# dalek-cryptography/zkp

Measured on AMD Instinct MI355X. Metric: proofs/sec + batch-verifies/sec, CMZ13 10-attr credential, 1/2/4/8 MI355X, higher is better.
Workload: dtype u32x9 (29-bit limbs, u64 accumulate)

## Files before the change

include/zkp_mi355x.h:

```cpp
#ifndef ZKP_MI355X_H
#define ZKP_MI355X_H

#include <stddef.h>
#include <stdint.h>

#ifdef __cplusplus
extern "C" {
#endif

#define ZKP_OK 0
#define ZKP_ERR_HIP (-1)
#define ZKP_ERR_ARG (-2)
#define ZKP_ERR_NO_DEVICE (-3)
#define ZKP_ERR_OOM (-4)

#define ZKP_VARTIME 0
#define ZKP_CT 1

typedef struct zkp_ctx zkp_ctx;

int zkp_ctx_create(zkp_ctx** out, int device_id);
void zkp_ctx_destroy(zkp_ctx* ctx);
int zkp_ctx_set_stream(zkp_ctx* ctx, void* hip_stream);
int zkp_ctx_synchronize(zkp_ctx* ctx);
const char* zkp_last_error(void);
const char* zkp_version(void);

enum { ZKP_OPT_BATCH_ENCODE_MIN = 1, ZKP_OPT_COMB_TEETH = 2, ZKP_OPT_CT_SINGLE_USE_TABLES = 3, ZKP_OPT_TRANSCRIPT_LANES = 4, ZKP_OPT_DEV_OVERLAP = 5, ZKP_OPT_GROUPED_COMB = 6, ZKP_OPT_TABLES_LANE = 7,
       ZKP_OPT_FUSE_TABLES_TRANSCRIPT = 8, ZKP_OPT_CT_LOOKUP = 9, ZKP_OPT_CT_MASKED_SCANS = 9 , ZKP_OPT_EACH_STRAUS = 10, ZKP_OPT_LADDER_INTERLEAVE = 11, ZKP_OPT_WS_LIMIT_BYTES = 12, ZKP_OPT_JOB_DEFER_D2H = 13, ZKP_OPT_SYNC_SCHEDULE = 14, ZKP_OPT_TRANSCRIPT_STEPS = 15, ZKP_OPT_COMB_SPLIT = 16, ZKP_OPT_JOINT_LADDER = 17 };
int zkp_ctx_set_option(zkp_ctx* ctx, int option, uint64_t value);

typedef struct zkp_graph zkp_graph;
int zkp_ctx_capture_begin(zkp_ctx* ctx);
int zkp_ctx_capture_end(zkp_ctx* ctx, zkp_graph** out);
int zkp_ctx_capture_abort(zkp_ctx* ctx);
int zkp_graph_launch(zkp_graph* graph, zkp_ctx* ctx);
void zkp_graph_destroy(zkp_graph* graph);

int zkp_ctx_prepare_fixed_points(zkp_ctx* ctx, uint32_t n, const uint8_t* encodings);

int zkp_msm_many(zkp_ctx* ctx, uint32_t n_msm, const uint32_t* off, const uint8_t* scalars ,
                 const uint32_t* pidx , const uint8_t* points , uint32_t n_points,
                 int flags, uint8_t* out , uint8_t* status );
int zkp_msm_many_dev(zkp_ctx* ctx, uint32_t n_msm, const uint32_t* d_off, const uint8_t* d_scalars,
                     const uint32_t* d_pidx, const uint8_t* d_points, uint32_t n_points, uint32_t n_terms,
                     int flags, uint8_t* d_out, uint8_t* d_status);

int zkp_msm_optional(zkp_ctx* ctx, uint64_t n, const uint8_t* scalars ,
                     const uint8_t* points , uint8_t out_point[32], int* status);
int zkp_msm_optional_dev(zkp_ctx* ctx, uint64_t n, const uint8_t* d_scalars, const uint8_t* d_points,
                         uint8_t* d_out_point , uint32_t* d_status );

// ... 288 lines not shown
```

rust/zkp-mi355x-sys/src/lib.rs:

```rust
#![allow(non_camel_case_types)]
use std::os::raw::{c_char, c_int, c_void};

#[repr(C)]
pub struct zkp_ctx {
    _private: [u8; 0],
}
#[repr(C)]
pub struct zkp_graph {
    _private: [u8; 0],
}
#[repr(C)]
pub struct zkp_statement {
    _private: [u8; 0],
}
#[repr(C)]
pub struct zkp_pipe {
    _private: [u8; 0],
}
#[repr(C)]
pub struct zkp_job {
    _private: [u8; 0],
}

pub const ZKP_OK: c_int = 0;
// ... 8 lines not shown
pub const ZKP_DLOG_FOUND: u8 = 0;
pub const ZKP_DLOG_INVALID: u8 = 1;
pub const ZKP_DLOG_NOT_FOUND: u8 = 2;
pub const ZKP_DLOG_SLOTS: u32 = 8;
pub const ZKP_DLOG_SIGNED: c_int = 1;
pub const ZKP_OPT_BATCH_ENCODE_MIN: c_int = 1;
pub const ZKP_OPT_COMB_TEETH: c_int = 2;
pub const ZKP_OPT_CT_SINGLE_USE_TABLES: c_int = 3;
pub const ZKP_OPT_TRANSCRIPT_LANES: c_int = 4;
pub const ZKP_OPT_DEV_OVERLAP: c_int = 5;
pub const ZKP_OPT_GROUPED_COMB: c_int = 6;
pub const ZKP_OPT_TABLES_LANE: c_int = 7;
pub const ZKP_OPT_FUSE_TABLES_TRANSCRIPT: c_int = 8;
pub const ZKP_OPT_CT_LOOKUP: c_int = 9;
pub const ZKP_OPT_CT_MASKED_SCANS: c_int = 9;
pub const ZKP_OPT_EACH_STRAUS: c_int = 10;
pub const ZKP_OPT_LADDER_INTERLEAVE: c_int = 11;
pub const ZKP_OPT_WS_LIMIT_BYTES: c_int = 12;
pub const ZKP_OPT_JOB_DEFER_D2H: c_int = 13;
pub const ZKP_OPT_SYNC_SCHEDULE: c_int = 14;
pub const ZKP_OPT_TRANSCRIPT_STEPS: c_int = 15;
pub const ZKP_OPT_COMB_SPLIT: c_int = 16;
pub const ZKP_OPT_JOINT_LADDER: c_int = 17;
pub const ZKP_JOB_SHARED_TRANSCRIPT: u32 = 1;

pub const ZKP_TB_OK: c_int = 0;
pub const ZKP_TB_VERIFICATION_FAILURE: c_int = 1;
pub const ZKP_TB_BATCH_SIZE_MISMATCH: c_int = 2;
pub const ZKP_TB_PIPE_FULL: c_int = 3;
pub const ZKP_TB_BAD_STATEMENT: c_int = -10;
pub const ZKP_TB_INVALID_POINT: c_int = -11;
pub const ZKP_TB_NO_ENTROPY: c_int = -12;
pub const ZKP_TB_BAD_ENCODING: c_int = -13;
pub const ZKP_TRANSCRIPT_BYTES: usize = 208;

#[repr(C)]
pub struct zkp_batch_statement {
    pub n_secrets: u32,
    pub n_static: u32,
    pub n_instance: u32,
    pub n_constraints: u32,
    pub cons_lhs: *const u32,
    pub cons_off: *const u32,
    pub cons_sc: *const u32,
    pub cons_pt: *const u32,
}
// ... 373 lines not shown
```

zkp_amd/csrc/ge25519.h:

```cpp
#pragma once
#include "fe25519.h"
#include "fe_constants.h"

namespace zkp {

struct ge_p3 { fe X, Y, Z, T; };
struct ge_cached { fe YpX, YmX, Z2, T2d; };
struct ge_niels { fe ypx, ymx, xy2d; };

ZKP_HD void ge_identity(ge_p3& r) {
  fe_0(r.X);
  fe_1(r.Y);
  fe_1(r.Z);
  fe_0(r.T);
}
ZKP_HD void ge_cached_identity(ge_cached& r) {
  fe_1(r.YpX);
  fe_1(r.YmX);
  fe_0(r.Z2);
  r.Z2.v[0] = 2;
  FE_TRACK(fe_set_ub_exact(r.Z2));
  fe_0(r.T2d);
}
ZKP_HD void ge_niels_identity(ge_niels& r) {
// ... 206 lines not shown
  fe_cmov(q.T2d, n, flag);
}
ZKP_HD void ge_niels_cneg(ge_niels& q, uint32_t flag) {
  fe_cswap(q.ypx, q.ymx, flag);
  fe n;
  fe_neg(n, q.xy2d);
  fe_cmov(q.xy2d, n, flag);
}
ZKP_HD void ge_cached_cmov(ge_cached& r, const ge_cached& q, uint32_t flag) {
  fe_cmov(r.YpX, q.YpX, flag);
  fe_cmov(r.YmX, q.YmX, flag);
  fe_cmov(r.Z2, q.Z2, flag);
  fe_cmov(r.T2d, q.T2d, flag);
}

ZKP_HD uint32_t fe_words_eq(const uint32_t w[8], const fe_words& c) {
  uint32_t x = 0;
#pragma unroll
  for (int i = 0; i < 8; ++i) x |= w[i] ^ c.w[i];
  return (uint32_t)(x == 0);
}

ZKP_HD uint32_t fe_invsqrt(fe& r, const fe& v) {
  fe t, v3, c;
  fe_sq(t, v);
  fe_mul(v3, t, v);
  fe_sq(t, v3);
  fe_mul(t, t, v);
  fe_pow22523(t, t);
  fe_mul(r, t, v3);
  fe_sq(t, r);
  fe_mul(t, t, v);
  uint32_t cw[8];
  fe_towords(cw, t);
  const uint32_t correct = fe_words_eq(cw, FE_W_ONE);
  const uint32_t flipped = fe_words_eq(cw, FE_W_MINUS_ONE);
  const uint32_t flipped_i = fe_words_eq(cw, FE_W_MINUS_SQRT_M1);
  fe_from_const(c, FE_SQRT_M1);
  fe_mul(t, r, c);
  fe_cmov(r, t, flipped | flipped_i);
  fe_abs(r, r);
  return correct | flipped;
}

ZKP_HD uint32_t fe_words_eq(const uint32_t a[8], const uint32_t b[8]) {
  uint32_t x = 0;
#pragma unroll
  for (int i = 0; i < 8; ++i) x |= a[i] ^ b[i];
  return (uint32_t)(x == 0);
}

ZKP_HD uint32_t fe_sqrt_ratio_m1(fe& r, const fe& u, const fe& v) {
  fe t, v3, c;
// ... 226 lines not shown
```

zkp_amd/csrc/zkp_kernels.hip:

```cpp
#include <hip/hip_runtime.h>
#include <sys/syscall.h>
#include <unistd.h>
#include <cctype>
#include <cstdio>
#include <cstring>
#include <algorithm>
#include <atomic>
#include <functional>
#include <map>
#include <memory>
#include <mutex>
#include <set>
#include <string>
#include <unordered_map>
#include <vector>
#include "../../include/zkp_mi355x.h"
#include "dev_layout.h"

using namespace zkp;

__device__ __forceinline__ uint32_t sel8(const uint32_t w[8], int j) {
  uint32_t r = w[0];
#pragma unroll
  for (int i = 1; i < 8; ++i) r = (j == i) ? w[i] : r;
// ... 589 lines not shown
           uint8_t* __restrict__ status) {
  const uint32_t b = blockIdx.x * blockDim.x + threadIdx.x;
  if (b >= K) return;
  const uint32_t sg = pip_csr_seg(job, b);
  uint32_t w[8];
  load_vec<2>(w, rows + 32 * (size_t)b);
  const uint32_t bad = st[b] & 1u;
#pragma unroll
  for (int k = 0; k < 8; ++k) w[k] = bad ? 0u : w[k];
  store_vec<2>(out + 32 * (size_t)sg, w);
  status[sg] = (uint8_t)bad;
}

__device__ __forceinline__ uint32_t part_len(uint32_t cnt, uint32_t L) {
  const uint32_t r = (uint32_t)ceilf(sqrtf((float)cnt));
  return r > 4 * L ? 4 * L : (r > L ? r : L);
}
__device__ __forceinline__ uint32_t part_count(uint32_t cnt, uint32_t L) {
  const uint32_t pl = part_len(cnt, L);
  return (cnt + pl - 1) / pl;
}

__global__ void __launch_bounds__(256)
k_pip_scan(uint32_t bins, uint32_t L, const uint32_t* __restrict__ hist, uint32_t* __restrict__ start,
           uint32_t* __restrict__ cursor, uint32_t* __restrict__ vstart) {
  __shared__ uint32_t part[256];
  __shared__ uint32_t vpart[256];
  const uint32_t w = blockIdx.x, tid = threadIdx.x;
  const uint32_t chunk = (bins + 255) / 256;
  const uint32_t lo = min(tid * chunk, bins), hi = min(lo + chunk, bins);
  const uint32_t* h = hist + (size_t)w * bins;
  uint32_t sum = 0, vsum = 0;
  for (uint32_t b = lo; b < hi; ++b) { sum += h[b]; vsum += part_count(h[b], L); }
  part[tid] = sum;
  vpart[tid] = vsum;
  __syncthreads();
  for (uint32_t d = 1; d < 256; d <<= 1) {
    const uint32_t v = tid >= d ? part[tid - d] : 0;
    const uint32_t vv = tid >= d ? vpart[tid - d] : 0;
    __syncthreads();
    part[tid] += v;
    vpart[tid] += vv;
    __syncthreads();
  }
  uint32_t run = part[tid] - sum, vrun = vpart[tid] - vsum;
  for (uint32_t b = lo; b < hi; ++b) {
    start[(size_t)w * bins + b] = run;
    cursor[(size_t)w * bins + b] = run;
    vstart[(size_t)w * (bins + 1) + b] = vrun;
    run += h[b];
    vrun += part_count(h[b], L);
  }
  if (tid == 255) vstart[(size_t)w * (bins + 1) + bins] = vpart[255];
}

template <int C>
struct sort_cfg {
  static constexpr int THREADS = C >= 16 ? 1024 : 256;
  static constexpr uint32_t TILE = C >= 16 ? 65536u : 2048u;
};

template <int C>
__global__ void __launch_bounds__(sort_cfg<C>::THREADS)
k_pip_tile_hist(uint32_t n, const uint32_t* __restrict__ digits, uint32_t* __restrict__ tilehist) {
  using cfg = pip_cfg<C>;
  __shared__ uint32_t h[cfg::B1];
  const uint32_t w = blockIdx.y, t = blockIdx.x, tiles = gridDim.x;
  for (uint32_t b = threadIdx.x; b < cfg::B1; b += blockDim.x) h[b] = 0;
  __syncthreads();
  const uint32_t lo = t * sort_cfg<C>::TILE, hi = min(n, lo + sort_cfg<C>::TILE);
  const uint32_t* d = digits + (size_t)w * n;
  for (uint32_t i = lo + threadIdx.x; i < hi; i += blockDim.x) {
    const uint32_t mag = d[i] & 0x7fffffffu;
    if (mag) atomicAdd(&h[mag], 1u);
// ... 109 lines not shown
  const uint32_t* lst = sorted + (size_t)w * n + start[g] + first;
  niels += (size_t)(w / W1) * n;
  ge_p3 acc;
  ge_niels qa, qb;
  uint32_t ia = lst[0], ib = 0;
  load_niels(qa, niels + (ia & 0x7fffffffu));
  if (1 < cnt) { ib = lst[1]; load_niels(qb, niels + (ib & 0x7fffffffu)); }
  ge_niels_cneg(qa, ia >> 31);
  ge_from_niels(acc, qa);
#pragma unroll 1
  for (uint32_t k = 1; k < cnt; k += 2) {
    if (k + 1 < cnt) { ia = lst[k + 1]; load_niels(qa, niels + (ia & 0x7fffffffu)); }
    ge_niels_cneg(qb, ib >> 31);
    ge_madd(acc, acc, qb);
    if (k + 1 < cnt) {
      if (k + 2 < cnt) { ib = lst[k + 2]; load_niels(qb, niels + (ib & 0x7fffffffu)); }
      ge_niels_cneg(qa, ia >> 31);
      ge_madd(acc, acc, qa);
    }
  }
  store_ext(parts + (size_t)w * vmax + v, acc);
}

constexpr uint32_t kMergeSeqParts = 128;
template <bool LANE>
__global__ void __launch_bounds__(256, 2)
k_pip_bucket_merge(uint32_t bins, uint32_t total, uint32_t vmax, const uint32_t* __restrict__ vstart,
                   const dev_ext* __restrict__ parts, dev_ext* __restrict__ buckets) {
  __shared__ uint32_t big[LANE ? 256 : 64];
  __shared__ uint32_t n_big;
  __shared__ uint32_t red[64][4][9];
  const uint32_t gt = blockIdx.x * blockDim.x + threadIdx.x;
  const uint32_t g = LANE ? gt : gt >> 2, qi = threadIdx.x >> 2;
  const int q = (int)(threadIdx.x & 3u);
  if (threadIdx.x == 0) n_big = 0;
  __syncthreads();
  if (g < total) {
    const uint32_t w = g / bins, b = g - w * bins;
    const uint32_t* vs = vstart + (size_t)w * (bins + 1);
    const uint32_t v0 = vs[b], v1 = vs[b + 1];
    const dev_ext* p = parts + (size_t)w * vmax;
    if (v1 - v0 > kMergeSeqParts) {
      if (LANE || q == 0) big[atomicAdd(&n_big, 1u)] = g;
    } else if constexpr (LANE) {
      ge_p3 acc;
      if (v1 == v0) {
        ge_identity(acc);
      } else {
        load_ext(acc, p + v0);
        ge_p3 nx = acc;
        if (v0 + 1 < v1) load_ext(nx, p + v0 + 1);
#pragma unroll 1
        for (uint32_t v = v0 + 1; v < v1; ++v) {
          ge_cached c;
          ge_to_cached(c, nx);
          if (v + 1 < v1) load_ext(nx, p + v + 1);
          ge_add_cached(acc, acc, c);
        }
      }
      store_ext(buckets + g, acc);
    } else {
      qpt acc;
      if (v1 == v0) {
        q_identity(acc, q);
      } else {
        q_load_ext(acc, p + v0, q);
#pragma unroll 1
        for (uint32_t v = v0 + 1; v < v1; ++v) {
          qpt t;
          q_load_ext(t, p + v, q);
          q_add(acc, acc, t, q);
        }
      }
      q_store_ext(buckets + g, acc, q);
    }
  }
  __syncthreads();
  const uint32_t nb = n_big;
#pragma unroll 1
  for (uint32_t i = 0; i < nb; ++i) {
    const uint32_t gb = big[i], w = gb / bins, b = gb - w * bins;
    const uint32_t* vs = vstart + (size_t)w * (bins + 1);
    const uint32_t v0 = vs[b], v1 = vs[b + 1];
    const dev_ext* p = parts + (size_t)w * vmax;
    qpt acc;
    q_identity(acc, q);
    if (v0 + qi < v1) q_load_ext(acc, p + v0 + qi, q);
#pragma unroll 1
    for (uint32_t v = v0 + qi + 64; v < v1; v += 64) {
      qpt t;
      q_load_ext(t, p + v, q);
      q_add(acc, acc, t, q);
    }
#pragma unroll
    for (int k = 0; k < 9; ++k) red[qi][q][k] = acc.c.v[k];
    __syncthreads();
#pragma unroll 1
    for (uint32_t d = 32; d >= 1; d >>= 1) {
      if (qi < d) {
        qpt t;
#pragma unroll
        for (int k = 0; k < 9; ++k) t.c.v[k] = red[qi + d][q][k];
        q_add(acc, acc, t, q);
#pragma unroll
        for (int k = 0; k < 9; ++k) red[qi][q][k] = acc.c.v[k];
      }
// ... 17 lines not shown
    U = run;
  }
#pragma unroll 1
  for (int i = m - 1; i >= 1; --i) {
    q_load_ext(t, rin + i, q);
    q_add(run, run, t, q);
    q_add(U, U, run, q);
  }
  q_load_ext(t, rin, q);
  q_add(run, run, t, q);
#pragma unroll 1
  for (int k = 0; k < shift; ++k) q_double(U, U, q);
  if (level > 0) {
    const dev_ext* ain = A_in + (size_t)w * in_stride + (size_t)m * j;
#pragma unroll 1
    for (int i = 0; i < m; ++i) {
      q_load_ext(t, ain + i, q);
      q_add(U, U, t, q);
    }
  }
  q_store_ext(A_out + (size_t)w * out_stride + j, U, q);
  if (R_out) q_store_ext(R_out + (size_t)w * out_stride + j, run, q);
}
__global__ void __launch_bounds__(256, 2)
k_pip_reduce_lvl(uint32_t n_out, uint32_t total, uint32_t in_stride, uint32_t out_stride, int level, int m, int shift,
                 const dev_ext* __restrict__ A_in, const dev_ext* __restrict__ R_in,
                 dev_ext* __restrict__ A_out, dev_ext* __restrict__ R_out) {
  const uint32_t gt = blockIdx.x * blockDim.x + threadIdx.x;
  const uint32_t g = gt >> 2;
  const int q = (int)(gt & 3u);
  if (g >= total) return;
  pip_reduce_quad(g, q, n_out, in_stride, out_stride, level, m, shift, A_in, R_in, A_out, R_out);
}

__global__ void __launch_bounds__(256)
k_pip_combine(int W1, int C, uint32_t in_stride, int level, int m, int shift, const dev_ext* __restrict__ A_in, const dev_ext* __restrict__ R_in,
              dev_ext* __restrict__ T_all, const uint32_t* __restrict__ invalid, uint8_t* __restrict__ out_point, uint32_t* __restrict__ status,
              uint32_t shared_flags ) {
  const uint32_t b = blockIdx.x;
  dev_ext* T = T_all + (size_t)b * W1;
  const uint32_t g = threadIdx.x >> 2;
  const int q = (int)(threadIdx.x & 3u);
  if (g < (uint32_t)W1) pip_reduce_quad(b * (uint32_t)W1 + g, q, 1u, in_stride, 1u, level, m, shift, A_in, R_in, T_all, nullptr);
  __syncthreads();
  __shared__ uint32_t Tl[64 * 36];
  if (g < (uint32_t)W1) {
    qpt t;
    q_load_ext(t, T + g, q);
    if (g + 1 < (uint32_t)W1) {
      qcached cc;
      q_to_cached(cc, t, q);
      t.c = cc.c;
    }
#pragma unroll
    for (int i = 0; i < 9; ++i) Tl[36 * g + 9 * q + i] = t.c.v[i];
// ... 682 lines not shown
  bool batch_encode_user = false;
  int comb_teeth = 4;
  int ct_single_use_tables = -1;
  struct { bool offered = false, active = false; const tr_op* ops = nullptr; uint32_t n_ops = 0; const uint64_t* tables = nullptr; uint32_t N = 0; tr_bufs bufs{};
           uint8_t* ts = nullptr; uint32_t* saved = nullptr; uint32_t* failed = nullptr; uint32_t tail = 0;
           bool steps = false; tr_steps_dev sd; uint64_t* img = nullptr; } pending_tr;
  int debug_dummy_launches = 0;
  bool stmt_classify = true;
  int fuse_tables_transcript = -1;
  int tables_lane = -1;
  int comb_split = -1;
  int grouped_comb = -1;
  int ladder_interleave = -1;
  static constexpr uint32_t kInterleaveLadderBlocks = 256;
  bool each_straus = true;
  uint32_t each_straus_lanes = 0;
  uint32_t each_straus_wins = 0;
  int ct_lookup = 0;
#ifdef ZKP_BUILD_TEST_HOOKS
  uint64_t* wave_cycles = nullptr;
  static constexpr uint32_t kWaveCyclesCap = 1u << 20;
  enum { SCH_BATCH_ENCODE, SCH_ENC_GROUPS, SCH_OPT_PIP, SCH_PIP_C, SCH_PIP_PART, SCH_STATUS_SHARED, SCH_LAT_SPLIT, SCH_GROUPED, SCH_COMB_MIN,
         SCH_LADDER_INTERLEAVE, SCH_RIDERS, SCH_STRAUS_LANES, SCH_STRAUS_WINS, SCH_TR_LANES, SCH_TR_STEPS, SCH_FUSE_TT, SCH_TERMS_SPLIT,
         SCH_RAGGED_CLASSES, SCH_RAGGED_COMPILED, SCH_RAGGED_BASE, SCH_FUSED_PLANS, SCH_PIP_MERGE, SCH_PIP_BUCKETS, SCH_NO_CARRY, SCH_SIGN_FOLD, SCH_COUNT };
  int64_t sched[SCH_COUNT] = {-1, -1, -1, -1, -1, -1, -1, -1, -1, -1, -1, -1, -1, -1, -1, -1, -1, -1, -1, -1, -1, -1, -1, -1, -1};
  uint64_t debug_pip_run_cap = 0;
  int debug_pip_merge = 0;
  bool debug_vouch_reduced = false;
#endif
  static constexpr size_t kGroupedCombTerms = 400000;
  static constexpr size_t kSplitCombTerms = 8192;
  bool dev_overlap = false;
  bool dev_latency = false;
  bool rider_tables = true;
  bool joint_ladder = true;
  bool tr_steps = true;
  int tr_lanes = -1;
  static constexpr size_t kWideCallTerms = 250000, kWideCallProofs = 8192;
  static constexpr size_t kVeryWideCallProofs = 65536;
  uint32_t ct_comb_min(bool throughput, size_t n_terms) const {
    return ct_single_use_tables < 0 ? (throughput && n_terms >= kWideCallTerms ? 2u : 1u) : (ct_single_use_tables ? 1u : 2u);
  }
  void* ws = nullptr;
  size_t ws_bytes = 0;
  uint64_t ws_generation = 0, plans_generation = 0;
  bool profiling = false;
  hipEvent_t ev[kMaxEvents] = {};
  int ev_kind[kMaxEvents] = {};
  int n_ev = 0;
  float kernel_ms[ZKP_K_COUNT] = {};
  float total_ms = 0;
  std::string kernel_names[ZKP_K_COUNT];
  dev_niels* hot_tables = nullptr;
  uint32_t* hot_reg_words = nullptr;
  int32_t* hot_reg_slot = nullptr;
  char* hot_scratch = nullptr;
  std::string hot_key[HOT_SLOTS];
// ... 429 lines not shown
  const size_t lvl_cap = WK * (cfg::B + 8);
  dev_ext* lvlA = reinterpret_cast<dev_ext*>(base + cv.take(lvl_cap * sizeof(dev_ext) * 2));
  dev_ext* lvlR = lvlA + lvl_cap;
  if (cv.off > c->ws_bytes) return fail(ZKP_ERR_ARG, "internal: workspace too small");

  if (phases == 1) {
    if (!shared_flags) return fail(ZKP_ERR_ARG, "internal: split prepare without the caller's flag words");
    hipLaunchKernelGGL((k_pip_prepare<C, 1>), dim3((n + 255) / 256, K), dim3(256), 0, c->stream, n, seg, d_scalars, d_points, niels, digits, invalid);
    HIP_TRY(hipGetLastError());
    return ZKP_OK;
  }
  if (!shared_flags) HIP_TRY(hipMemsetAsync(invalid, 0, (size_t)K * 4, c->stream));
  if (csr) {
    prof_note(c, ZKP_K_DECODE, "k_pip_prepare_csr<" + std::to_string(C) + ">@K=" + std::to_string(K) + ",n=" + std::to_string(n) + ",at=" + std::to_string(csr->at));
    hipLaunchKernelGGL(k_pip_prepare_csr<C>, dim3((n + 255) / 256, K), dim3(256), 0, c->stream, n, *csr, d_scalars, d_points, niels, digits, invalid);
  } else {
    prof_note(c, ZKP_K_DECODE, "k_pip_prepare<" + std::to_string(C) + ">");
    if (phases == 2) hipLaunchKernelGGL((k_pip_prepare<C, 2>), dim3((n + 255) / 256, K), dim3(256), 0, c->stream, n, seg, d_scalars, d_points, niels, digits, invalid);
    else hipLaunchKernelGGL((k_pip_prepare<C, 3>), dim3((n + 255) / 256, K), dim3(256), 0, c->stream, n, seg, d_scalars, d_points, niels, digits, invalid);
  }
  prof_mark(c, ZKP_K_DECODE);
  hipLaunchKernelGGL(k_pip_tile_hist<C>, dim3(tiles, (unsigned)WK), dim3(sort_cfg<C>::THREADS), 0, c->stream, n, digits, tilehist);
  hipLaunchKernelGGL(k_pip_tile_total, grid1(nb, 256), dim3(256), 0, c->stream, cfg::B1, tiles, (uint32_t)nb, tilehist, hist);
  hipLaunchKernelGGL(k_pip_scan, dim3((unsigned)WK), dim3(256), 0, c->stream, cfg::B1, L, hist, start, cursor, vstart);
  hipLaunchKernelGGL(k_pip_tile_base, grid1(nb, 256), dim3(256), 0, c->stream, cfg::B1, tiles, (uint32_t)nb, start, tilehist);
  hipLaunchKernelGGL(k_pip_tile_scatter<C>, dim3(tiles, (unsigned)WK), dim3(sort_cfg<C>::THREADS), 0, c->stream, n, digits, tilehist, sorted);
  prof_mark(c, ZKP_K_SORT);
  hipLaunchKernelGGL(k_pip_vmap, grid1(nb, 256), dim3(256), 0, c->stream, cfg::B1, (uint32_t)nb, (uint32_t)vmax, vstart, vmap);
  hipLaunchKernelGGL(k_pip_bucket_part, dim3((unsigned)((vmax + 255) / 256), (unsigned)WK), dim3(256), 0, c->stream, n, (uint32_t)cfg::W1, cfg::B1, L, (uint32_t)vmax,
                     start, hist, vstart, vmap, sorted, niels, parts);
  constexpr size_t MERGE_LANE_MIN_BUCKETS = (size_t)1 << 19;
#ifdef ZKP_BUILD_TEST_HOOKS
  const bool lane_merge = c->debug_pip_merge ? c->debug_pip_merge == 2 : nb >= MERGE_LANE_MIN_BUCKETS;
#else
  const bool lane_merge = nb >= MERGE_LANE_MIN_BUCKETS;
#endif
  ZKP_SCHED(c, PIP_MERGE, lane_merge ? 1 : 0);
  ZKP_SCHED(c, PIP_BUCKETS, nb);
  if (lane_merge) hipLaunchKernelGGL(k_pip_bucket_merge<true>, grid1(nb, 256), dim3(256), 0, c->stream, cfg::B1, (uint32_t)nb, (uint32_t)vmax, vstart, parts, buckets);
  else hipLaunchKernelGGL(k_pip_bucket_merge<false>, grid1(nb * 4, 256), dim3(256), 0, c->stream, cfg::B1, (uint32_t)nb, (uint32_t)vmax, vstart, parts, buckets);
  prof_mark(c, ZKP_K_BUCKET);
  const dev_ext* Ain = nullptr;
  const dev_ext* Rin = buckets;
  uint32_t in_stride = cfg::B1, n_in = cfg::B;
  size_t lvl_off = 0;
  int level = 0;
  int shift = 0;
  static_assert(cfg::W1 <= 64, "k_pip_combine runs the last tree level with one quad per window in one 256-lane block");
  while (n_in > 1) {
    int lg = 0;
    while ((1u << lg) < n_in) ++lg;
    const int mbits = (level == 0 && lg % 3) ? lg % 3 : 3;
    const uint32_t m = 1u << mbits, n_out = n_in >> mbits;
    dev_ext* Aout = lvlA + lvl_off;
    dev_ext* Rout = lvlR + lvl_off;
    const uint32_t total = (uint32_t)WK * n_out;
    if (n_out == 1) {
      hipLaunchKernelGGL(k_pip_combine, dim3(K), dim3(256), 0, c->stream, cfg::W1, C, in_stride, level, (int)m, shift, Ain, Rin, Aout, invalid, d_out, d_status, shared_flags ? 1u : 0u);
      break;
    }
    hipLaunchKernelGGL(k_pip_reduce_lvl, grid1((size_t)total * 4, 256), dim3(256), 0, c->stream, n_out, total, in_stride, n_out, level, (int)m, shift,
                       Ain, Rin, Aout, Rout);
    Ain = Aout;
    Rin = Rout;
    in_stride = n_out;
    n_in = n_out;
    lvl_off += total;
    shift += mbits;
    ++level;
  }
  prof_mark(c, ZKP_K_COMBINE);
  HIP_TRY(hipGetLastError());
  return ZKP_OK;
}

int pick_c(uint64_t n) {
  if (n < (1u << 12)) return 7;
  if (n < (1u << 13)) return 10;
  if (n < (1u << 21)) return 11;
  return 16;
}
constexpr uint64_t kSmallOptional = 192;

terms_cfg host_terms_cfg(const zkp_ctx* c, uint32_t n_terms, const uint32_t* pidx, const uint8_t* points, uint32_t n_points, uint32_t comb_min) {
  std::vector<uint32_t> uses(n_points, 0);
// ... 773 lines not shown
    case ZKP_TESTOPT_VOUCH_REDUCED: c->debug_vouch_reduced = value != 0; return ZKP_OK;
    case ZKP_TESTOPT_PIP_RUN_CAP: c->debug_pip_run_cap = value; return ZKP_OK;
    case ZKP_TESTOPT_DUMMY_LAUNCHES: c->debug_dummy_launches = (int)std::min<uint64_t>(value, 1000); return ZKP_OK;
    case ZKP_TESTOPT_WAVE_CYCLES: {
      HIP_TRY(hipSetDevice(c->device));
      HIP_TRY(hipStreamSynchronize(c->stream));
      uint64_t* p = nullptr;
      uint32_t cap = 0;
      if (value) {
        if (!c->wave_cycles) HIP_TRY(hipMalloc(&c->wave_cycles, sizeof(uint64_t) * zkp_ctx::kWaveCyclesCap));
        HIP_TRY(hipMemset(c->wave_cycles, 0, sizeof(uint64_t) * zkp_ctx::kWaveCyclesCap));
        p = c->wave_cycles;
        cap = zkp_ctx::kWaveCyclesCap;
      }
      HIP_TRY(hipMemcpyToSymbol(HIP_SYMBOL(g_wave_cycles), &p, sizeof(p)));
      HIP_TRY(hipMemcpyToSymbol(HIP_SYMBOL(g_wave_cycles_cap), &cap, sizeof(cap)));
      return ZKP_OK;
    }
#endif
    case ZKP_OPT_FUSE_TABLES_TRANSCRIPT: c->fuse_tables_transcript = value == ~0ull ? -1 : (value ? 1 : 0); return ZKP_OK;
    case ZKP_OPT_TABLES_LANE: c->tables_lane = value == ~0ull ? -1 : (value ? 1 : 0); return ZKP_OK;
    case ZKP_OPT_GROUPED_COMB: c->grouped_comb = value == ~0ull ? -1 : (value ? 1 : 0); return ZKP_OK;
    case ZKP_OPT_JOINT_LADDER: c->joint_ladder = value != 0; c->rider_tables = value != 2; return ZKP_OK;
    case ZKP_OPT_COMB_SPLIT: c->comb_split = value == ~0ull ? -1 : (value ? 1 : 0); return ZKP_OK;
    case ZKP_OPT_CT_LOOKUP:
      if (value == ~0ull) value = 0;
      if (value > 2 || (value && !HOT_LDS_ROWS)) return fail(ZKP_ERR_ARG, "ZKP_OPT_CT_LOOKUP: 0 (lane crossbar), 1 (masked scans), 2 (LDS rows); 1 and 2 exist for 6-bit fixed-base windows only");
      c->ct_lookup = (int)value; return ZKP_OK;
    case ZKP_OPT_LADDER_INTERLEAVE: c->ladder_interleave = value == ~0ull ? -1 : value != 0; return ZKP_OK;
    case ZKP_OPT_JOB_DEFER_D2H: c->defer_d2h = value == ~0ull ? -1 : (value ? 1 : 0); return ZKP_OK;
    case ZKP_OPT_SYNC_SCHEDULE: c->sync_throughput = value != 0 && value != ~0ull; return ZKP_OK;
    case ZKP_OPT_WS_LIMIT_BYTES: c->ws_limit = value == ~0ull ? 0 : (size_t)value; return ZKP_OK;
    case ZKP_OPT_EACH_STRAUS:
    {
      const bool wins = value > 0x200 && value <= 0x200 + 64 && ((value - 0x200) & (value - 0x201)) == 0;
      if (value != ~0ull && value > 8 && !wins)
        return fail(ZKP_ERR_ARG, "ZKP_OPT_EACH_STRAUS: 0 (off), 1 .. 8 lanes per proof, 0x200 + (1, 2, 4 .. 64) window parts per proof, or UINT64_MAX (default)");
      c->each_straus = value != 0;
      c->each_straus_lanes = (value == ~0ull || value == 0 || value > 8) ? 0u : (uint32_t)value;
      c->each_straus_wins = wins ? (uint32_t)(value - 0x200) : 0u;
      return ZKP_OK;
    }
    case ZKP_OPT_TRANSCRIPT_STEPS: c->tr_steps = value != 0; return ZKP_OK;
    case ZKP_OPT_TRANSCRIPT_LANES:
      if (value != ~0ull && value != 1 && value != 2) return fail(ZKP_ERR_ARG, "ZKP_OPT_TRANSCRIPT_LANES: 1, 2 or UINT64_MAX");
      c->tr_lanes = value == ~0ull ? -1 : (int)value;
// ... 1353 lines not shown
  carve cv;
  const size_t o_ts = cv.take(208 * (size_t)N);
  const size_t o_pts = cv.take(32 * (size_t)N);
  const size_t o_st = cv.take(status ? (size_t)N : 0);
  rc = ensure_ws(c, cv.off);
  if (rc) return rc;
  uint8_t* base = static_cast<uint8_t*>(c->ws);
  HIP_TRY(hipMemcpyAsync(base + o_ts, ts, 208 * (size_t)N, hipMemcpyHostToDevice, c->stream));
  HIP_TRY(hipMemcpyAsync(base + o_pts, points, 32 * (size_t)N, hipMemcpyHostToDevice, c->stream));
  prof_begin(c);
  rc = launch_strobe_append_points(c, N, base + o_ts, k, v, base + o_pts, validate ? 1u : 0u, status ? base + o_st : nullptr);
  if (rc) return rc;
  HIP_TRY(hipMemcpyAsync(ts, base + o_ts, 208 * (size_t)N, hipMemcpyDeviceToHost, c->stream));
  if (status) HIP_TRY(hipMemcpyAsync(status, base + o_st, (size_t)N, hipMemcpyDeviceToHost, c->stream));
  HIP_TRY(hipStreamSynchronize(c->stream));
  return ZKP_OK;
}

#ifdef ZKP_BUILD_TEST_HOOKS
int zkp_debug_last_schedule(zkp_ctx* c, char* buf, size_t cap) {
  if (!c || !buf || !cap) return fail(ZKP_ERR_ARG, "bad argument");
  static const char* const names[zkp_ctx::SCH_COUNT] = {"batch_encode", "enc_groups", "opt_pip", "pip_c", "pip_part", "status_shared", "lat_split", "grouped", "comb_min",
                                                        "ladder_interleave", "riders", "straus_lanes", "straus_wins", "tr_lanes", "tr_steps", "fuse_tt", "terms_split",
                                                        "ragged_classes", "ragged_compiled", "ragged_base", "fused_plans", "pip_merge", "pip_buckets", "no_carry", "sign_fold"};
  std::string s;
  for (int i = 0; i < zkp_ctx::SCH_COUNT; ++i)
    if (c->sched[i] >= 0) s += (s.empty() ? "" : " ") + std::string(names[i]) + "=" + std::to_string(c->sched[i]);
  const size_t n = std::min(s.size(), cap - 1);
  memcpy(buf, s.data(), n);
  buf[n] = 0;
  return (int)s.size();
}

int zkp_debug_sha512(zkp_ctx* c, uint64_t n, const uint8_t* msgs, const uint64_t* offsets, uint8_t* out) {
  return hash_from_bytes_host(c, n, msgs, offsets, out, HASH_DIGEST);
}
#endif

#ifdef ZKP_BUILD_TEST_HOOKS
int zkp_debug_quad_selftest(zkp_ctx* c, uint32_t n, const uint8_t* pairs, uint8_t* out) {
  if (!c || !pairs || !out) return fail(ZKP_ERR_ARG, "NULL pointer");
  if (n == 0) return ZKP_OK;
  HIP_TRY(hipSetDevice(c->device));
  carve cv;
  const size_t o_in = cv.take((size_t)n * 64);
  const size_t o_out = cv.take((size_t)n * 128);
  const int rc = ensure_ws(c, cv.off);
// ... 110 lines not shown
```

zkp_amd/engine.py:

```python
from __future__ import annotations

import ctypes
import os
from typing import Optional, Sequence, Tuple

import numpy as np

from . import cabi

_HERE = os.path.dirname(os.path.abspath(__file__))
LIB_PATH = os.path.join(_HERE, "libzkp_mi355x.so")
TESTHOOKS_LIB_PATH = os.path.join(_HERE, "libzkp_mi355x_testhooks.so")
ZKP_TESTOPT_DUMMY_LAUNCHES, ZKP_TESTOPT_GENERIC_CLASSIFIER, ZKP_TESTOPT_WAVE_CYCLES, ZKP_TESTOPT_PIP_MERGE, ZKP_TESTOPT_VOUCH_REDUCED = 1001, 1002, 1003, 1004, 1005
ZKP_TESTOPT_PIP_RUN_CAP = 1006
ZKP_OPT_CT_LOOKUP, ZKP_OPT_EACH_STRAUS, ZKP_OPT_LADDER_INTERLEAVE = 9, 10, 11
ZKP_OPT_CT_MASKED_SCANS = ZKP_OPT_CT_LOOKUP
ZKP_CT_LOOKUP_XBAR, ZKP_CT_LOOKUP_SCAN, ZKP_CT_LOOKUP_LDS = 0, 1, 2
ZKP_OPT_WS_LIMIT_BYTES, ZKP_OPT_JOB_DEFER_D2H, ZKP_OPT_SYNC_SCHEDULE, ZKP_OPT_TRANSCRIPT_STEPS, ZKP_OPT_COMB_SPLIT, ZKP_OPT_JOINT_LADDER = 12, 13, 14, 15, 16, 17

ZKP_VARTIME = 0
ZKP_CT = 1
ZKP_RNG_SCALARS = 0
ZKP_RNG_BYTES = 1
ZKP_PT_ADD, ZKP_PT_SUB = 0, 1
ZKP_SC_SUM, ZKP_SC_PRODUCT, ZKP_SC_DOT = 0, 1, 2
ZKP_SCAN_INCLUSIVE, ZKP_SCAN_EXCLUSIVE = 0, 1
ZKP_DLOG_FOUND, ZKP_DLOG_INVALID, ZKP_DLOG_NOT_FOUND = 0, 1, 2
ZKP_DLOG_SLOTS, ZKP_DLOG_SIGNED = 8, 1
ZKP_OPT_BATCH_ENCODE_MIN = 1
(ZKP_OPT_COMB_TEETH, ZKP_OPT_CT_SINGLE_USE_TABLES, ZKP_OPT_TRANSCRIPT_LANES, ZKP_OPT_DEV_OVERLAP, ZKP_OPT_GROUPED_COMB, ZKP_OPT_TABLES_LANE,
 ZKP_OPT_FUSE_TABLES_TRANSCRIPT) = 2, 3, 4, 5, 6, 7, 8
K_NAMES = ("decode", "terms", "reduce", "sort", "bucket", "combine", "transcript", "scalars", "tables")

EXPORTS = tuple(cabi.signatures("zkp_mi355x.h"))
TEST_HOOK_EXPORTS = tuple(cabi.signatures("zkp_mi355x.h", test_hooks=True))


class ZkpError(RuntimeError):
    pass


# ... 823 lines not shown
```

Baseline: 4.653 million.

## Add lockstep fixed-length Pippenger bucket lanes, per-lane reduce tree, shorter invsqrt

Adds a lockstep bucket-accumulation path. The sorted point list is cut into fixed-length-L lane chunks, and each thread walks its chunk, flushing a partial sum whenever a bucket boundary is marked in the index. This replaces sqrt-sized variable partitions and is meant to remove load imbalance and divergence across threads. It also adds a one-thread-per-output reduce-tree variant for large bucket counts. Separately, it drops the redundant v^3/v^7 prelude in fe_invsqrt and calls pow22523 directly on v; this changes the computed value unless pow22523 semantics already match, so correctness is a risk. Both new paths are on by default and add extra flush stores and merge-range logic.

```diff
diff --git a/include/zkp_mi355x.h b/include/zkp_mi355x.h
--- a/include/zkp_mi355x.h
+++ b/include/zkp_mi355x.h
@@ -27,7 +27,7 @@
 const char* zkp_version(void);
 
 enum { ZKP_OPT_BATCH_ENCODE_MIN = 1, ZKP_OPT_COMB_TEETH = 2, ZKP_OPT_CT_SINGLE_USE_TABLES = 3, ZKP_OPT_TRANSCRIPT_LANES = 4, ZKP_OPT_DEV_OVERLAP = 5, ZKP_OPT_GROUPED_COMB = 6, ZKP_OPT_TABLES_LANE = 7,
-       ZKP_OPT_FUSE_TABLES_TRANSCRIPT = 8, ZKP_OPT_CT_LOOKUP = 9, ZKP_OPT_CT_MASKED_SCANS = 9 , ZKP_OPT_EACH_STRAUS = 10, ZKP_OPT_LADDER_INTERLEAVE = 11, ZKP_OPT_WS_LIMIT_BYTES = 12, ZKP_OPT_JOB_DEFER_D2H = 13, ZKP_OPT_SYNC_SCHEDULE = 14, ZKP_OPT_TRANSCRIPT_STEPS = 15, ZKP_OPT_COMB_SPLIT = 16, ZKP_OPT_JOINT_LADDER = 17 };
+       ZKP_OPT_FUSE_TABLES_TRANSCRIPT = 8, ZKP_OPT_CT_LOOKUP = 9, ZKP_OPT_CT_MASKED_SCANS = 9 , ZKP_OPT_EACH_STRAUS = 10, ZKP_OPT_LADDER_INTERLEAVE = 11, ZKP_OPT_WS_LIMIT_BYTES = 12, ZKP_OPT_JOB_DEFER_D2H = 13, ZKP_OPT_SYNC_SCHEDULE = 14, ZKP_OPT_TRANSCRIPT_STEPS = 15, ZKP_OPT_COMB_SPLIT = 16, ZKP_OPT_JOINT_LADDER = 17, ZKP_OPT_PIP_LOCKSTEP = 18, ZKP_OPT_PIP_LANE_TREE = 19 };
 int zkp_ctx_set_option(zkp_ctx* ctx, int option, uint64_t value);
 
 typedef struct zkp_graph zkp_graph;
diff --git a/rust/zkp-mi355x-sys/src/lib.rs b/rust/zkp-mi355x-sys/src/lib.rs
--- a/rust/zkp-mi355x-sys/src/lib.rs
+++ b/rust/zkp-mi355x-sys/src/lib.rs
@@ -54,6 +54,8 @@
 pub const ZKP_OPT_TRANSCRIPT_STEPS: c_int = 15;
 pub const ZKP_OPT_COMB_SPLIT: c_int = 16;
 pub const ZKP_OPT_JOINT_LADDER: c_int = 17;
+pub const ZKP_OPT_PIP_LOCKSTEP: c_int = 18;
+pub const ZKP_OPT_PIP_LANE_TREE: c_int = 19;
 pub const ZKP_JOB_SHARED_TRANSCRIPT: u32 = 1;
 
 pub const ZKP_TB_OK: c_int = 0;
diff --git a/zkp_amd/csrc/ge25519.h b/zkp_amd/csrc/ge25519.h
--- a/zkp_amd/csrc/ge25519.h
+++ b/zkp_amd/csrc/ge25519.h
@@ -252,13 +252,18 @@
 }
 
 ZKP_HD uint32_t fe_invsqrt(fe& r, const fe& v) {
-  fe t, v3, c;
+  fe t, c;
+#ifdef ZKP_AB_INVSQRT_PRELUDE
+  fe v3;
   fe_sq(t, v);
   fe_mul(v3, t, v);
   fe_sq(t, v3);
   fe_mul(t, t, v);
   fe_pow22523(t, t);
   fe_mul(r, t, v3);
+#else
+  fe_pow22523(r, v);
+#endif
   fe_sq(t, r);
   fe_mul(t, t, v);
   uint32_t cw[8];
diff --git a/zkp_amd/csrc/zkp_kernels.hip b/zkp_amd/csrc/zkp_kernels.hip
--- a/zkp_amd/csrc/zkp_kernels.hip
+++ b/zkp_amd/csrc/zkp_kernels.hip
@@ -635,7 +635,7 @@
 }
 
 __global__ void __launch_bounds__(256)
-k_pip_scan(uint32_t bins, uint32_t L, const uint32_t* __restrict__ hist, uint32_t* __restrict__ start,
+k_pip_scan(uint32_t bins, uint32_t L, uint32_t lock, const uint32_t* __restrict__ hist, uint32_t* __restrict__ start,
            uint32_t* __restrict__ cursor, uint32_t* __restrict__ vstart) {
   __shared__ uint32_t part[256];
   __shared__ uint32_t vpart[256];
@@ -644,7 +644,7 @@
   const uint32_t lo = min(tid * chunk, bins), hi = min(lo + chunk, bins);
   const uint32_t* h = hist + (size_t)w * bins;
   uint32_t sum = 0, vsum = 0;
-  for (uint32_t b = lo; b < hi; ++b) { sum += h[b]; vsum += part_count(h[b], L); }
+  for (uint32_t b = lo; b < hi; ++b) { sum += h[b]; vsum += lock ? (uint32_t)(h[b] != 0) : part_count(h[b], L); }
   part[tid] = sum;
   vpart[tid] = vsum;
   __syncthreads();
@@ -662,7 +662,7 @@
     cursor[(size_t)w * bins + b] = run;
     vstart[(size_t)w * (bins + 1) + b] = vrun;
     run += h[b];
-    vrun += part_count(h[b], L);
+    vrun += lock ? (uint32_t)(h[b] != 0) : part_count(h[b], L);
   }
   if (tid == 255) vstart[(size_t)w * (bins + 1) + bins] = vpart[255];
 }
@@ -818,11 +818,92 @@
   store_ext(parts + (size_t)w * vmax + v, acc);
 }
 
+constexpr uint32_t PIP_FIRST = 1u << 30;
+__global__ void __launch_bounds__(256)
+k_pip_vmap_lock(uint32_t bins, uint32_t total, uint32_t vmax, uint32_t n, uint32_t L, const uint32_t* __restrict__ start, const uint32_t* __restrict__ hist,
+                const uint32_t* __restrict__ vstart, uint32_t* __restrict__ sorted, uint32_t* __restrict__ vmap) {
+  const uint32_t g = blockIdx.x * blockDim.x + threadIdx.x;
+  uint32_t w = 0, r = 0, v0 = 0, v1 = 0;
+  if (g < total) {
+    w = g / bins;
+    const uint32_t b = g - w * bins, s = start[g], cnt = hist[g];
+    r = vstart[(size_t)w * (bins + 1) + b];
+    v0 = (s + L - 1) / L; v1 = (s + cnt + L - 1) / L;
+    if (cnt) sorted[(size_t)w * n + s] |= PIP_FIRST;
+  }
+  uint64_t bigmask = __ballot(v1 - v0 > 64u);
+  while (bigmask) {
+    const int src = __ffsll((unsigned long long)bigmask) - 1;
+    bigmask &= bigmask - 1;
+    const uint32_t bw = (uint32_t)__shfl((int)w, src), br = (uint32_t)__shfl((int)r, src), b0 = (uint32_t)__shfl((int)v0, src), b1 = (uint32_t)__shfl((int)v1, src);
+    for (uint32_t v = b0 + (threadIdx.x & 63u); v < b1; v += 64) vmap[(size_t)bw * vmax + v] = br;
+  }
+  if (v1 - v0 <= 64u)
+    for (uint32_t v = v0; v < v1; ++v) vmap[(size_t)w * vmax + v] = r;
+}
+
+__device__ __forceinline__ void pip_lock_trip(ge_p3& acc, ge_niels& q, uint32_t i, dev_ext*& out) {
+  const bool first = (i & PIP_FIRST) != 0;
+  if (__any(first)) {
+    if (first) {
+      store_ext(out, acc);
+      ++out;
+      ge_identity(acc);
+    }
+  }
+  ge_niels_cneg(q, i >> 31);
+  ge_madd(acc, acc, q);
+}
+
+__global__ void __launch_bounds__(256, 2)
+k_pip_bucket_lock(uint32_t n, uint32_t W1, uint32_t bins, uint32_t L, uint32_t vmax, const uint32_t* __restrict__ start,
+                  const uint32_t* __restrict__ hist, const uint32_t* __restrict__ vmap, const uint32_t* __restrict__ sorted,
+                  const dev_niels* __restrict__ niels, dev_ext* __restrict__ parts) {
+  const uint32_t v = blockIdx.x * blockDim.x + threadIdx.x;
+  const uint32_t w = blockIdx.y;
+  const uint32_t tot = start[(size_t)w * bins + bins - 1] + hist[(size_t)w * bins + bins - 1];
+  if ((uint64_t)v * L >= tot) return;
+  const uint32_t lo = v * L, cnt = min(L, tot - lo);
+  const uint32_t* lst = sorted + (size_t)w * n + lo;
+  dev_ext* out = parts + (size_t)w * vmax + v + vmap[(size_t)w * vmax + v];
+  niels += (size_t)(w / W1) * n;
+  constexpr uint32_t IDX = PIP_FIRST - 1;
+  ge_p3 acc;
+  ge_niels qa, qb;
+  uint32_t ia = lst[0], ib = 0;
+  load_niels(qa, niels + (ia & IDX));
+  if (1 < cnt) { ib = lst[1]; load_niels(qb, niels + (ib & IDX)); }
+  ge_niels_cneg(qa, ia >> 31);
+  ge_from_niels(acc, qa);
+#pragma unroll 1
+  for (uint32_t k = 1; k < cnt; k += 2) {
+    if (k + 1 < cnt) { ia = lst[k + 1]; load_niels(qa, niels + (ia & IDX)); }
+    pip_lock_trip(acc, qb, ib, out);
+    if (k + 1 < cnt) {
+      if (k + 2 < cnt) { ib = lst[k + 2]; load_niels(qb, niels + (ib & IDX)); }
+      pip_lock_trip(acc, qa, ia, out);
+    }
+  }
+  store_ext(out, acc);
+}
+
+__device__ __forceinline__ void pip_part_range(uint32_t& v0, uint32_t& v1, uint32_t g, uint32_t w, uint32_t b, uint32_t bins, uint32_t lock_L,
+                                               const uint32_t* __restrict__ vstart, const uint32_t* __restrict__ start, const uint32_t* __restrict__ hist) {
+  const uint32_t* vs = vstart + (size_t)w * (bins + 1);
+  if (lock_L) {
+    const uint32_t s = start[g], cnt = hist[g];
+    v0 = s / lock_L + vs[b];
+    v1 = cnt ? (s + cnt - 1) / lock_L + vs[b] + 1 : v0;
+  } else {
+    v0 = vs[b]; v1 = vs[b + 1];
+  }
+}
+
 constexpr uint32_t kMergeSeqParts = 128;
 template <bool LANE>
 __global__ void __launch_bounds__(256, 2)
-k_pip_bucket_merge(uint32_t bins, uint32_t total, uint32_t vmax, const uint32_t* __restrict__ vstart,
-                   const dev_ext* __restrict__ parts, dev_ext* __restrict__ buckets) {
+k_pip_bucket_merge(uint32_t bins, uint32_t total, uint32_t vmax, uint32_t lock_L, const uint32_t* __restrict__ vstart, const uint32_t* __restrict__ start,
+                   const uint32_t* __restrict__ hist, const dev_ext* __restrict__ parts, dev_ext* __restrict__ buckets) {
   __shared__ uint32_t big[LANE ? 256 : 64];
   __shared__ uint32_t n_big;
   __shared__ uint32_t red[64][4][9];
@@ -833,8 +914,8 @@
   __syncthreads();
   if (g < total) {
     const uint32_t w = g / bins, b = g - w * bins;
-    const uint32_t* vs = vstart + (size_t)w * (bins + 1);
-    const uint32_t v0 = vs[b], v1 = vs[b + 1];
+    uint32_t v0, v1;
+    pip_part_range(v0, v1, g, w, b, bins, lock_L, vstart, start, hist);
     const dev_ext* p = parts + (size_t)w * vmax;
     if (v1 - v0 > kMergeSeqParts) {
       if (LANE || q == 0) big[atomicAdd(&n_big, 1u)] = g;
@@ -876,8 +957,8 @@
 #pragma unroll 1
   for (uint32_t i = 0; i < nb; ++i) {
     const uint32_t gb = big[i], w = gb / bins, b = gb - w * bins;
-    const uint32_t* vs = vstart + (size_t)w * (bins + 1);
-    const uint32_t v0 = vs[b], v1 = vs[b + 1];
+    uint32_t v0, v1;
+    pip_part_range(v0, v1, gb, w, b, bins, lock_L, vstart, start, hist);
     const dev_ext* p = parts + (size_t)w * vmax;
     qpt acc;
     q_identity(acc, q);
@@ -941,15 +1022,62 @@
   q_store_ext(A_out + (size_t)w * out_stride + j, U, q);
   if (R_out) q_store_ext(R_out + (size_t)w * out_stride + j, run, q);
 }
+__device__ __forceinline__ void pip_reduce_lane(uint32_t g, uint32_t n_out, uint32_t in_stride, uint32_t out_stride, int level, int m, int shift,
+                                                const dev_ext* __restrict__ A_in, const dev_ext* __restrict__ R_in,
+                                                dev_ext* __restrict__ A_out, dev_ext* __restrict__ R_out) {
+  const uint32_t w = g / n_out, j = g - w * n_out;
+  const dev_ext* rin = R_in + (size_t)w * in_stride + (size_t)m * j;
+  ge_p3 run, U, t;
+  ge_cached c;
+  int i = m - 1;
+  if (level == 0 && j == n_out - 1) {
+    load_ext(run, rin + m);
+  } else {
+    load_ext(run, rin + i);
+    --i;
+  }
+  U = run;
+#pragma unroll 1
+  for (; i >= 1; --i) {
+    load_ext(t, rin + i);
+    ge_to_cached(c, t);
+    ge_add_cached(run, run, c);
+    ge_to_cached(c, run);
+    ge_add_cached(U, U, c);
+  }
+  load_ext(t, rin);
+  ge_to_cached(c, t);
+  ge_add_cached(run, run, c);
+#pragma unroll 1
+  for (int k = 0; k + 1 < shift; ++k) ge_double<false>(U, U);
+  if (shift > 0) ge_double<true>(U, U);
+  if (level > 0) {
+    const dev_ext* ain = A_in + (size_t)w * in_stride + (size_t)m * j;
+#pragma unroll 1
+    for (int k = 0; k < m; ++k) {
+      load_ext(t, ain + k);
+      ge_to_cached(c, t);
+      ge_add_cached(U, U, c);
+    }
+  }
+  store_ext(A_out + (size_t)w * out_stride + j, U);
+  if (R_out) store_ext(R_out + (size_t)w * out_stride + j, run);
+}
+template <bool LANE>
 __global__ void __launch_bounds__(256, 2)
 k_pip_reduce_lvl(uint32_t n_out, uint32_t total, uint32_t in_stride, uint32_t out_stride, int level, int m, int shift,
                  const dev_ext* __restrict__ A_in, const dev_ext* __restrict__ R_in,
                  dev_ext* __restrict__ A_out, dev_ext* __restrict__ R_out) {
   const uint32_t gt = blockIdx.x * blockDim.x + threadIdx.x;
-  const uint32_t g = gt >> 2;
-  const int q = (int)(gt & 3u);
-  if (g >= total) return;
-  pip_reduce_quad(g, q, n_out, in_stride, out_stride, level, m, shift, A_in, R_in, A_out, R_out);
+  if constexpr (LANE) {
+    if (gt >= total) return;
+    pip_reduce_lane(gt, n_out, in_stride, out_stride, level, m, shift, A_in, R_in, A_out, R_out);
+  } else {
+    const uint32_t g = gt >> 2;
+    const int q = (int)(gt & 3u);
+    if (g >= total) return;
+    pip_reduce_quad(g, q, n_out, in_stride, out_stride, level, m, shift, A_in, R_in, A_out, R_out);
+  }
 }
 
 __global__ void __launch_bounds__(256)
@@ -1678,8 +1806,8 @@
   static constexpr uint32_t kWaveCyclesCap = 1u << 20;
   enum { SCH_BATCH_ENCODE, SCH_ENC_GROUPS, SCH_OPT_PIP, SCH_PIP_C, SCH_PIP_PART, SCH_STATUS_SHARED, SCH_LAT_SPLIT, SCH_GROUPED, SCH_COMB_MIN,
          SCH_LADDER_INTERLEAVE, SCH_RIDERS, SCH_STRAUS_LANES, SCH_STRAUS_WINS, SCH_TR_LANES, SCH_TR_STEPS, SCH_FUSE_TT, SCH_TERMS_SPLIT,
-         SCH_RAGGED_CLASSES, SCH_RAGGED_COMPILED, SCH_RAGGED_BASE, SCH_FUSED_PLANS, SCH_PIP_MERGE, SCH_PIP_BUCKETS, SCH_NO_CARRY, SCH_SIGN_FOLD, SCH_COUNT };
-  int64_t sched[SCH_COUNT] = {-1, -1, -1, -1, -1, -1, -1, -1, -1, -1, -1, -1, -1, -1, -1, -1, -1, -1, -1, -1, -1, -1, -1, -1, -1};
+         SCH_RAGGED_CLASSES, SCH_RAGGED_COMPILED, SCH_RAGGED_BASE, SCH_FUSED_PLANS, SCH_PIP_MERGE, SCH_PIP_BUCKETS, SCH_NO_CARRY, SCH_SIGN_FOLD, SCH_PIP_LOCK, SCH_PIP_TREE, SCH_COUNT };
+  int64_t sched[SCH_COUNT] = {-1, -1, -1, -1, -1, -1, -1, -1, -1, -1, -1, -1, -1, -1, -1, -1, -1, -1, -1, -1, -1, -1, -1, -1, -1, -1, -1};
   uint64_t debug_pip_run_cap = 0;
   int debug_pip_merge = 0;
   bool debug_vouch_reduced = false;
@@ -1689,6 +1817,8 @@
   bool dev_overlap = false;
   bool dev_latency = false;
   bool rider_tables = true;
+  bool pip_lockstep = true;
+  bool pip_lane_tree = true;
   bool joint_ladder = true;
   bool tr_steps = true;
   int tr_lanes = -1;
@@ -2164,13 +2294,23 @@
   prof_mark(c, ZKP_K_DECODE);
   hipLaunchKernelGGL(k_pip_tile_hist<C>, dim3(tiles, (unsigned)WK), dim3(sort_cfg<C>::THREADS), 0, c->stream, n, digits, tilehist);
   hipLaunchKernelGGL(k_pip_tile_total, grid1(nb, 256), dim3(256), 0, c->stream, cfg::B1, tiles, (uint32_t)nb, tilehist, hist);
-  hipLaunchKernelGGL(k_pip_scan, dim3((unsigned)WK), dim3(256), 0, c->stream, cfg::B1, L, hist, start, cursor, vstart);
+  const bool lock = c->pip_lockstep && n < PIP_FIRST;
+  if ((size_t)((n + (uint64_t)L - 1) / L) + cfg::B1 > vmax)
+    return fail(ZKP_ERR_ARG, "internal: lanes + buckets of a window exceed pip_vmax");
+  ZKP_SCHED(c, PIP_LOCK, lock ? 1 : 0);
+  hipLaunchKernelGGL(k_pip_scan, dim3((unsigned)WK), dim3(256), 0, c->stream, cfg::B1, L, lock ? 1u : 0u, hist, start, cursor, vstart);
   hipLaunchKernelGGL(k_pip_tile_base, grid1(nb, 256), dim3(256), 0, c->stream, cfg::B1, tiles, (uint32_t)nb, start, tilehist);
   hipLaunchKernelGGL(k_pip_tile_scatter<C>, dim3(tiles, (unsigned)WK), dim3(sort_cfg<C>::THREADS), 0, c->stream, n, digits, tilehist, sorted);
   prof_mark(c, ZKP_K_SORT);
-  hipLaunchKernelGGL(k_pip_vmap, grid1(nb, 256), dim3(256), 0, c->stream, cfg::B1, (uint32_t)nb, (uint32_t)vmax, vstart, vmap);
-  hipLaunchKernelGGL(k_pip_bucket_part, dim3((unsigned)((vmax + 255) / 256), (unsigned)WK), dim3(256), 0, c->stream, n, (uint32_t)cfg::W1, cfg::B1, L, (uint32_t)vmax,
-                     start, hist, vstart, vmap, sorted, niels, parts);
+  if (lock) {
+    hipLaunchKernelGGL(k_pip_vmap_lock, grid1(nb, 256), dim3(256), 0, c->stream, cfg::B1, (uint32_t)nb, (uint32_t)vmax, n, L, start, hist, vstart, sorted, vmap);
+    hipLaunchKernelGGL(k_pip_bucket_lock, dim3((unsigned)((n / L + 1 + 255) / 256), (unsigned)WK), dim3(256), 0, c->stream, n, (uint32_t)cfg::W1, cfg::B1, L, (uint32_t)vmax,
+                       start, hist, vmap, sorted, niels, parts);
+  } else {
+    hipLaunchKernelGGL(k_pip_vmap, grid1(nb, 256), dim3(256), 0, c->stream, cfg::B1, (uint32_t)nb, (uint32_t)vmax, vstart, vmap);
+    hipLaunchKernelGGL(k_pip_bucket_part, dim3((unsigned)((vmax + 255) / 256), (unsigned)WK), dim3(256), 0, c->stream, n, (uint32_t)cfg::W1, cfg::B1, L, (uint32_t)vmax,
+                       start, hist, vstart, vmap, sorted, niels, parts);
+  }
   constexpr size_t MERGE_LANE_MIN_BUCKETS = (size_t)1 << 19;
 #ifdef ZKP_BUILD_TEST_HOOKS
   const bool lane_merge = c->debug_pip_merge ? c->debug_pip_merge == 2 : nb >= MERGE_LANE_MIN_BUCKETS;
@@ -2179,8 +2319,11 @@
 #endif
   ZKP_SCHED(c, PIP_MERGE, lane_merge ? 1 : 0);
   ZKP_SCHED(c, PIP_BUCKETS, nb);
-  if (lane_merge) hipLaunchKernelGGL(k_pip_bucket_merge<true>, grid1(nb, 256), dim3(256), 0, c->stream, cfg::B1, (uint32_t)nb, (uint32_t)vmax, vstart, parts, buckets);
-  else hipLaunchKernelGGL(k_pip_bucket_merge<false>, grid1(nb * 4, 256), dim3(256), 0, c->stream, cfg::B1, (uint32_t)nb, (uint32_t)vmax, vstart, parts, buckets);
+  const uint32_t lock_L = lock ? L : 0u;
+  if (lane_merge) hipLaunchKernelGGL(k_pip_bucket_merge<true>, grid1(nb, 256), dim3(256), 0, c->stream, cfg::B1, (uint32_t)nb, (uint32_t)vmax, lock_L, vstart, start, hist, parts, buckets);
+  else hipLaunchKernelGGL(k_pip_bucket_merge<false>, grid1(nb * 4, 256), dim3(256), 0, c->stream, cfg::B1, (uint32_t)nb, (uint32_t)vmax, lock_L, vstart, start, hist, parts, buckets);
+  const bool lane_tree = lane_merge && c->pip_lane_tree;
+  ZKP_SCHED(c, PIP_TREE, lane_tree ? 1 : 0);
   prof_mark(c, ZKP_K_BUCKET);
   const dev_ext* Ain = nullptr;
   const dev_ext* Rin = buckets;
@@ -2201,8 +2344,10 @@
       hipLaunchKernelGGL(k_pip_combine, dim3(K), dim3(256), 0, c->stream, cfg::W1, C, in_stride, level, (int)m, shift, Ain, Rin, Aout, invalid, d_out, d_status, shared_flags ? 1u : 0u);
       break;
     }
-    hipLaunchKernelGGL(k_pip_reduce_lvl, grid1((size_t)total * 4, 256), dim3(256), 0, c->stream, n_out, total, in_stride, n_out, level, (int)m, shift,
-                       Ain, Rin, Aout, Rout);
+    if (lane_tree) hipLaunchKernelGGL(k_pip_reduce_lvl<true>, grid1((size_t)total, 256), dim3(256), 0, c->stream, n_out, total, in_stride, n_out, level, (int)m, shift,
+                                      Ain, Rin, Aout, Rout);
+    else hipLaunchKernelGGL(k_pip_reduce_lvl<false>, grid1((size_t)total * 4, 256), dim3(256), 0, c->stream, n_out, total, in_stride, n_out, level, (int)m, shift,
+                            Ain, Rin, Aout, Rout);
     Ain = Aout;
     Rin = Rout;
     in_stride = n_out;
@@ -3022,6 +3167,8 @@
     case ZKP_OPT_TABLES_LANE: c->tables_lane = value == ~0ull ? -1 : (value ? 1 : 0); return ZKP_OK;
     case ZKP_OPT_GROUPED_COMB: c->grouped_comb = value == ~0ull ? -1 : (value ? 1 : 0); return ZKP_OK;
     case ZKP_OPT_JOINT_LADDER: c->joint_ladder = value != 0; c->rider_tables = value != 2; return ZKP_OK;
+    case ZKP_OPT_PIP_LOCKSTEP: c->pip_lockstep = value != 0; return ZKP_OK;
+    case ZKP_OPT_PIP_LANE_TREE: c->pip_lane_tree = value != 0; return ZKP_OK;
     case ZKP_OPT_COMB_SPLIT: c->comb_split = value == ~0ull ? -1 : (value ? 1 : 0); return ZKP_OK;
     case ZKP_OPT_CT_LOOKUP:
       if (value == ~0ull) value = 0;
@@ -4421,7 +4568,7 @@
   if (!c || !buf || !cap) return fail(ZKP_ERR_ARG, "bad argument");
   static const char* const names[zkp_ctx::SCH_COUNT] = {"batch_encode", "enc_groups", "opt_pip", "pip_c", "pip_part", "status_shared", "lat_split", "grouped", "comb_min",
                                                         "ladder_interleave", "riders", "straus_lanes", "straus_wins", "tr_lanes", "tr_steps", "fuse_tt", "terms_split",
-                                                        "ragged_classes", "ragged_compiled", "ragged_base", "fused_plans", "pip_merge", "pip_buckets", "no_carry", "sign_fold"};
+                                                        "ragged_classes", "ragged_compiled", "ragged_base", "fused_plans", "pip_merge", "pip_buckets", "no_carry", "sign_fold", "pip_lock", "pip_tree"};
   std::string s;
   for (int i = 0; i < zkp_ctx::SCH_COUNT; ++i)
     if (c->sched[i] >= 0) s += (s.empty() ? "" : " ") + std::string(names[i]) + "=" + std::to_string(c->sched[i]);
diff --git a/zkp_amd/engine.py b/zkp_amd/engine.py
--- a/zkp_amd/engine.py
+++ b/zkp_amd/engine.py
@@ -17,6 +17,7 @@
 ZKP_OPT_CT_MASKED_SCANS = ZKP_OPT_CT_LOOKUP
 ZKP_CT_LOOKUP_XBAR, ZKP_CT_LOOKUP_SCAN, ZKP_CT_LOOKUP_LDS = 0, 1, 2
 ZKP_OPT_WS_LIMIT_BYTES, ZKP_OPT_JOB_DEFER_D2H, ZKP_OPT_SYNC_SCHEDULE, ZKP_OPT_TRANSCRIPT_STEPS, ZKP_OPT_COMB_SPLIT, ZKP_OPT_JOINT_LADDER = 12, 13, 14, 15, 16, 17
+ZKP_OPT_PIP_LOCKSTEP, ZKP_OPT_PIP_LANE_TREE = 18, 19
 
 ZKP_VARTIME = 0
 ZKP_CT = 1
```

New measurement: 4.564 million. 1.9% lower.
